# cloneofsimo/vqgan-training

Hardware: AMD Instinct MI355X
Metric: images/sec full train step (enc+dec+LPIPS+disc+bwd), 256x256 f=8 (higher is better)
Workload: dtype mixed like the reference: encoder+LPIPS+discriminator fp16 operands (TF32's 10-bit mantissa) / fp32 accumulate, decoder bf16

## Files before the change

### vqgan-training_amd/csrc/conv_wgrad.hip

```cpp
#include "vq_common.h"

struct WgradParams {
  VqConvDesc d;
  const void* x;
  const void* dy;
  float* part;
  float* bias_part;
  int dbg;
  int M, HoWo, RS;
  int n_ct, n_cit;
  int dsh, ush;
  int pix_per_split;
  int nsplit;
  int xcd_tiles;
  int wo_shift, ho_shift;
  int seg_shift;
  int x3;
};

#ifdef VQ_STAMPS_ON
__device__ long long g_vq_wstamps[64];
__device__ int g_vq_wstamp_n;
#define VQ_WSTAMP(id) do { if (blockIdx.x == 0 && threadIdx.x == 0) { const long long t_ = (long long)__builtin_readcyclecounter(); \
    const int k_ = g_vq_wstamp_n; if (k_ < 64) { g_vq_wstamps[k_] = ((long long)(id) << 56) | (t_ & 0x00ffffffffffffffll); g_vq_wstamp_n = k_ + 1; } } } while (0)
// ... 297 lines not shown
#pragma unroll
  for (int e = 0; e < 8; ++e) ones[e] = (short)One16<DT>::BITS;
#pragma unroll
  for (int e = 0; e < 16; ++e) bacc[e] = 0.f;

  const int gg = lane >> 4, tl = lane & 15;
  const int frow = 8 * (gg >> 1) + (tl >> 2);
  const int fcol = (gg & 1) * 16 + (tl & 3) * 4;
  auto frag_addr = [&](int chan0) -> int {
    const int c = chan0 + fcol;
    const int seg = (c * 2) >> 6, within = (c * 2) & 63;
    return frow * RB + ((seg ^ seg_key(frow)) << 6) + within;
  };
  auto frag_addr_x3 = [&](int chan0, int plane) -> int {
    const int c = chan0 + ((fcol >> 3) << 4) + (fcol & 7);
    const int seg = (c * 2) >> 6, within = ((c * 2) & 63) ^ ((seg & 1) << 4);
    return (frow * RB + ((seg ^ seg_key(frow)) << 6) + within) ^ (plane << 4);
  };
  int ya[FRC], xa[FRI];
#pragma unroll
  for (int a = 0; a < FRC; ++a) ya[a] = X3 ? frag_addr_x3(wco + (a >> 1) * 64, a & 1) : frag_addr(wco + a * 32);
#pragma unroll
  for (int b = 0; b < FRI; ++b) xa[b] = TILE * 2 + (X3 ? frag_addr_x3(wci + (b >> 1) * 64, b & 1) : frag_addr(wci + b * 32));
  constexpr int NRD = 2 * (FRC + FRI);
  static_assert(NRD <= 15, "lgkmcnt is a 4-bit counter");

  constexpr bool DB = BT < 256;
  auto run = [&](auto bias_tag) {
    constexpr bool BIAS = decltype(bias_tag)::value;
    s16x4 fy[DB ? 2 : 1][FRC][2], fx[DB ? 2 : 1][FRI][2];
    auto issue = [&](const char* base, auto kk_tag, int slot) {
      constexpr int KOFF = decltype(kk_tag)::value * 16 * RB;
#pragma unroll
      for (int a = 0; a < FRC; ++a) {
        fy[slot][a][0] = lds_read_tr16_b64_async<KOFF>(base + ya[a]);
        fy[slot][a][1] = lds_read_tr16_b64_async<KOFF + 4 * RB>(base + ya[a]);
      }
#pragma unroll
      for (int b = 0; b < FRI; ++b) {
        fx[slot][b][0] = lds_read_tr16_b64_async<KOFF>(base + xa[b]);
        fx[slot][b][1] = lds_read_tr16_b64_async<KOFF + 4 * RB>(base + xa[b]);
      }
    };
    auto mma = [&](int slot) {
#pragma unroll
      for (int a = 0; a < FRC; ++a)
#pragma unroll
        for (int h = 0; h < 2; ++h) vq_tie(fy[slot][a][h]);
#pragma unroll
      for (int b = 0; b < FRI; ++b)
#pragma unroll
        for (int h = 0; h < 2; ++h) vq_tie(fx[slot][b][h]);
      s16x8 af[FRC], bfr[FRI];
#pragma unroll
      for (int a = 0; a < FRC; ++a)
#pragma unroll
        for (int e = 0; e < 4; ++e) { af[a][e] = fy[slot][a][0][e]; af[a][4 + e] = fy[slot][a][1][e]; }
#pragma unroll
      for (int b = 0; b < FRI; ++b)
#pragma unroll
        for (int e = 0; e < 4; ++e) { bfr[b][e] = fx[slot][b][0][e]; bfr[b][4 + e] = fx[slot][b][1][e]; }
      if constexpr (X3) {
#pragma unroll
        for (int a = 0; a < AFR; ++a)
#pragma unroll
          for (int b = 0; b < BFR; ++b) {
            acc[a][b] = mfma16<DT>(af[2 * a], bfr[2 * b], acc[a][b]);
            acc[a][b] = mfma16<DT>(af[2 * a], bfr[2 * b + 1], acc[a][b]);
            acc[a][b] = mfma16<DT>(af[2 * a + 1], bfr[2 * b], acc[a][b]);
          }
        if constexpr (BIAS) {
          s16x8 selh = af[0], sell = af[1];
#pragma unroll
          for (int a = 1; a < AFR; ++a)
#pragma unroll
            for (int e = 0; e < 8; ++e) { selh[e] = (bias_frag == a) ? af[2 * a][e] : selh[e]; sell[e] = (bias_frag == a) ? af[2 * a + 1][e] : sell[e]; }
          bacc = mfma16<DT>(selh, ones, bacc);
          bacc = mfma16<DT>(sell, ones, bacc);
        }
      } else {
#pragma unroll
        for (int a = 0; a < FRC; ++a)
#pragma unroll
          for (int b = 0; b < FRI; ++b) acc[a][b] = mfma16<DT>(af[a], bfr[b], acc[a][b]);
        if constexpr (BIAS) {
          s16x8 sel = af[0];
#pragma unroll
          for (int a = 1; a < FRC; ++a)
#pragma unroll
            for (int e = 0; e < 8; ++e) sel[e] = (bias_frag == a) ? af[a][e] : sel[e];
          bacc = mfma16<DT>(sel, ones, bacc);
        }
      }
    };
    stage(0);
    wait_vmcnt<0>();
    raw_barrier();
    for (int c = 0; c < nchunks; ++c) {
      const char* base = (const char*)(lds + (c & 1) * 2 * TILE);
      issue(base, std::integral_constant<int, 0>{}, 0);
#ifdef VQ_ABLATION_KERNELS
      if (c + 1 < nchunks && !(p.dbg & 1)) stage((c + 1) & 1);
#else
      if (c + 1 < nchunks) stage((c + 1) & 1);
#endif
      if constexpr (DB) {
        issue(base, std::integral_constant<int, 1>{}, 1);
        wait_lgkmcnt<NRD>(); mma(0);
        issue(base, std::integral_constant<int, 2>{}, 0);
        wait_lgkmcnt<NRD>(); mma(1);
        issue(base, std::integral_constant<int, 3>{}, 1);
        wait_lgkmcnt<NRD>(); mma(0);
        wait_lgkmcnt<0>(); mma(1);
      } else {
        wait_lgkmcnt<0>(); mma(0);
        issue(base, std::integral_constant<int, 1>{}, 0);
        wait_lgkmcnt<0>(); mma(0);
        issue(base, std::integral_constant<int, 2>{}, 0);
        wait_lgkmcnt<0>(); mma(0);
        issue(base, std::integral_constant<int, 3>{}, 0);
        wait_lgkmcnt<0>(); mma(0);
      }
      wait_vmcnt<0>();
      raw_barrier();
    }
  };
  if (nchunks > 0) {
    if (do_bias) run(std::true_type{});
    else run(std::false_type{});
  }

  const int fr = lane & 31, fh = lane >> 5;
  const int CoutS = X3 ? p.d.Cout / 2 : p.d.Cout, CinS = X3 ? p.d.Cin / 2 : p.d.Cin;
  const int cob = X3 ? (co0 + wco) / 2 : co0 + wco, cib = X3 ? (ci0 + wci) / 2 : ci0 + wci;
  if (do_bias && (wave % NWI) == 0 && fr == 0) {
#pragma unroll
    for (int e = 0; e < 16; ++e)
      p.bias_part[(int64_t)split * CoutS + cob + bias_frag * 32 + (e & 3) + 8 * (e >> 2) + 4 * fh] = bacc[e];
  }
  float* out = p.part + ((int64_t)(split * p.RS + tap) * CoutS) * CinS;
#pragma unroll
  for (int a = 0; a < AFR; ++a)
#pragma unroll
    for (int b = 0; b < BFR; ++b) {
      const int ci = cib + b * 32 + fr;
#pragma unroll
      for (int e = 0; e < 16; ++e) {
        const int co = cob + a * 32 + (e & 3) + 8 * (e >> 2) + 4 * fh;
        wg_store(p, &out[(int64_t)co * CinS + ci], acc[a][b][e]);
      }
    }
}

template <int DT, int GEN, int NW, int SEG = 0, int STAG = 0, int X3 = 0>
__global__ __launch_bounds__(NW * 64, 2) void conv_wgrad3_kernel(const WgradParams p) {
  constexpr int BT = 128, BKP = 64, RB = BT * 2, XROWS = GEN ? 96 : 72;
  static_assert(GEN ? SEG == 0 : (SEG >= 4 && SEG <= 6), "SEG: compile-time segment shift of the power-of-two form");
  static_assert(!X3 || (NW == 4 && DT == VQ_F16), "the native three-product form: 2 x 2 waves over binary16 pieces");
  constexpr int TILE_Y = BKP * BT, TILE_X = XROWS * BT, STAGE = TILE_Y + TILE_X;
  constexpr int NWI = NW / 2, WTI = BT / NWI;
  constexpr int FRC = 2, FRI = WTI / 32;
  constexpr int AFR = X3 ? 1 : FRC, BFR = X3 ? 1 : FRI;
  constexpr int BXOR = X3 ? 4 : 6;
  static_assert(!X3 || FRI == 2, "native form: 64 virtual = 32 real channels per wave and side");
  constexpr int YP = (BKP / 4) / NW;
  constexpr int XPT = XROWS / 4, XP = (XPT + NW - 1) / NW;
  static_assert(NW == 4 || NW == 8, "2 x 2 or 2 x 4 waves");
  VQ_DYN_LDS(vq_bf16, lds);

  const int tid = threadIdx.x, lane = tid & 63, wave = tid >> 6;
  VQ_WSTAMP(20);
  const int wco = (wave / NWI) * 64, wci = (wave % NWI) * WTI;
  const int tiles = 3 * p.n_cit * p.n_ct;
  const int xcd = blockIdx.x & 7, jb = blockIdx.x >> 3;
  int split, t;
  if (p.xcd_tiles == 2) {
    const int per = (int)(gridDim.x >> 3), idx = xcd * per + jb;
    if (idx >= p.nsplit * tiles) return;
    split = idx / tiles;
    t = idx - split * tiles;
  } else if (p.xcd_tiles) {
    const int tpx = tiles >> 3;
    t = xcd * tpx + jb % tpx;
    split = jb / tpx;
  } else {
    split = (jb / tiles) * 8 + xcd;
    t = jb % tiles;
  }
  if (split >= p.nsplit) return;
  const int kr = t % 3; t /= 3;
  const int cit = t % p.n_cit; const int ct = t / p.n_cit;
  const int co0 = ct * BT, ci0 = cit * BT;
  const int pbeg = split * p.pix_per_split;
  int pend = pbeg + p.pix_per_split;
  if (pend > p.M) pend = p.M;
  const int nchunks = pbeg < pend ? (pend - pbeg + BKP - 1) / BKP : 0;

  const int W = p.d.Wo, H = p.d.Ho;
  const int wsh = p.wo_shift, hsh = p.ho_shift, wmask = W - 1, hmask = H - 1;
  constexpr bool pow2 = !GEN;
  const int segsh = GEN ? p.seg_shift : SEG;
  const int wseg = 1 << segsh, nslots = (BKP >> segsh) * (wseg + 2);
  const vq_bf16* zero = (const vq_bf16*)g_vq_wg_zero_page;
  const vq_bf16* dyb = (const vq_bf16*)p.dy;
  const vq_bf16* xb = (const vq_bf16*)p.x;

  const int lrow = lane >> 4, lp = lane & 15;
  auto lsl_of = [&](int row) -> int {
    const int seg = (lp >> 2) ^ (row & 3), gr = (lp & 3) ^ (X3 ? (seg & 1) : 0);
    return ((seg << 2) | gr) << 3;
  };
  const vq_bf16* pdy0 = dyb + (int64_t)(pbeg + wave * 4 + lrow) * p.d.Cout + co0 + lsl_of(lrow);
  const int dy_piece = 4 * NW * p.d.Cout;
  int xqj[GEN ? XP : 1];
  const int xlsl = lsl_of(lrow);
  if constexpr (GEN) {
#pragma unroll
    for (int i = 0; i < XP; ++i) {
      const int slot = (wave + NW * i) * 4 + lrow;
      const int q = slot / (wseg + 2);
      xqj[i] = slot < nslots ? ((q << 8) | (slot - q * (wseg + 2))) : -1;
    }
  }
  const int cin0 = ci0 + xlsl;
  int m0 = pbeg;
  auto stage = [&](int buf) {
    vq_bf16* ybase = lds + buf * STAGE;
    vq_bf16* xbase = ybase + TILE_Y;
#pragma unroll
    for (int i = 0; i < YP; ++i) glds16(pdy0 + i * dy_piece, ybase + (wave + NW * i) * 4 * BT);
    pdy0 += (int64_t)BKP * p.d.Cout;
#pragma unroll
    for (int i = 0; i < XP; ++i) {
      if (wave + NW * i < XPT) {
        int q, jj;
        bool have;
        if constexpr (GEN) { q = xqj[i] >> 8; jj = xqj[i] & 255; have = xqj[i] >= 0; }
        else {
          constexpr int WS2 = (1 << SEG) + 2;
          const int slot = (wave + NW * i) * 4 + lrow;
          q = slot / WS2; jj = slot - q * WS2; have = slot < (BKP >> SEG) * WS2;
        }
        const int ms = m0 + (q << segsh);
        int ox0, oy, n;
        if constexpr (pow2) { ox0 = ms & wmask; oy = (ms >> wsh) & hmask; n = ms >> (wsh + hsh); }
        else { n = ms / p.HoWo; const int rem = ms - n * p.HoWo; oy = rem / W; ox0 = rem - oy * W; }
        const int iy = oy + kr - 1, ix = ox0 - 1 + jj;
        const bool ok = have && (unsigned)iy < (unsigned)H && (unsigned)ix < (unsigned)W;
        const int off = ((n * p.d.H + (iy >> p.ush)) * p.d.W + (ix >> p.ush)) * p.d.Cin + cin0;
        const vq_bf16* src = ok ? xb + off : zero + xlsl;
        glds16((const void*)src, xbase + (wave + NW * i) * 4 * BT);
      }
    }
    m0 += BKP;
  };

  const int gg = lane >> 4, tl = lane & 15;
  const int frow = 8 * (gg >> 1) + (tl >> 2);
  const int fcol = (gg & 1) * 16 + (tl & 3) * 4;
  const int fcolv = X3 ? ((fcol >> 3) << 4) + (fcol & 7) : fcol;
  int ya[FRC];
#pragma unroll
  for (int a = 0; a < FRC; ++a) {
    const int c = wco + (X3 ? 0 : a * 32) + fcolv, seg = (c * 2) >> 6, within = ((c * 2) & 63) ^ (X3 ? ((seg & 1) << 4) : 0);
    ya[a] = (frow * RB + ((seg ^ (frow & 3)) << 6) + within) ^ (X3 ? (a << 4) : 0);
  }
  int xoff[GEN ? 4 : 1][GEN ? 3 : 1][GEN ? 2 : 1];
  int xsw[GEN ? 1 : 4];
  {
    const int c = wci + fcolv, seg = (c * 2) >> 6, within = ((c * 2) & 63) ^ (X3 ? ((seg & 1) << 4) : 0);
    if constexpr (GEN) {
#pragma unroll
      for (int kk = 0; kk < 4; ++kk)
#pragma unroll
        for (int ks = 0; ks < 3; ++ks)
#pragma unroll
          for (int h = 0; h < 2; ++h) {
            const int r = kk * 16 + frow + 4 * h;
            const int row = r + 2 * (r >> segsh) + ks;
            xoff[kk][ks][h] = TILE_Y * 2 + row * RB + ((seg ^ (row & 3)) << 6) + within;
          }
    } else {
#pragma unroll
      for (int j = 0; j < 4; ++j) xsw[j] = TILE_Y * 2 + frow * RB + ((seg ^ ((frow + j) & 3)) << 6) + within;
    }
  }

  f32x16 acc[3][AFR][BFR];
#pragma unroll
  for (int ks = 0; ks < 3; ++ks)
#pragma unroll
    for (int a = 0; a < AFR; ++a)
#pragma unroll
      for (int b = 0; b < BFR; ++b)
#pragma unroll
        for (int e = 0; e < 16; ++e) acc[ks][a][b][e] = 0.f;
  const bool do_bias = p.bias_part != nullptr && cit == 0 && kr < AFR;
  auto store_bias = [&](const f32x16& bacc) {
    const int fr_ = lane & 31, fh_ = lane >> 5;
    if ((wave % NWI) == 0 && fr_ == 0) {
      const int cob = X3 ? (co0 + wco) / 2 : co0 + wco + kr * 32, cstride = X3 ? p.d.Cout / 2 : p.d.Cout;
#pragma unroll
      for (int e = 0; e < 16; ++e)
        p.bias_part[(int64_t)split * cstride + cob + (e & 3) + 8 * (e >> 2) + 4 * fh_] = bacc[e];
    }
  };

  auto run = [&](auto bias_tag) {
    constexpr bool BIAS = decltype(bias_tag)::value;
    f32x16 bacc;
    s16x8 ones;
    if constexpr (BIAS) {
#pragma unroll
      for (int e = 0; e < 8; ++e) ones[e] = (short)One16<DT>::BITS;
#pragma unroll
      for (int e = 0; e < 16; ++e) bacc[e] = 0.f;
    }
    constexpr int NX = 2;
    s16x4 fy[2][FRC][2], fx[NX][FRI][2];
    auto issue_y = [&](const char* base, auto kk_tag) {
      constexpr int KK = decltype(kk_tag)::value, KOFF = KK * 16 * RB;
#pragma unroll
      for (int a = 0; a < FRC; ++a) {
        fy[KK & 1][a][0] = lds_read_tr16_b64_async<KOFF>(base + ya[a]);
        fy[KK & 1][a][1] = lds_read_tr16_b64_async<KOFF + 4 * RB>(base + ya[a]);
      }
    };
    auto issue_x = [&](const char* base, auto u_tag) {
      constexpr int U = decltype(u_tag)::value, KK = U / 3, KS = U % 3;
#pragma unroll
      for (int b = 0; b < FRI; ++b) {
        if constexpr (GEN) {
          fx[U % NX][b][0] = lds_read_tr16_b64_async<0>(base + (xoff[KK][KS][0] ^ (b << BXOR)));
          fx[U % NX][b][1] = lds_read_tr16_b64_async<0>(base + (xoff[KK][KS][1] ^ (b << BXOR)));
        } else {
          constexpr int UR = 16 * KK + 2 * (KK >> (SEG - 4)) + KS;
          fx[U % NX][b][0] = lds_read_tr16_b64_async<UR * RB>(base + (xsw[UR & 3] ^ (b << BXOR)));
          fx[U % NX][b][1] = lds_read_tr16_b64_async<(UR + 4) * RB>(base + (xsw[UR & 3] ^ (b << BXOR)));
        }
      }
    };
    auto step = [&](const char* base, auto u_tag) {
      constexpr int U = decltype(u_tag)::value, KK = U / 3, KS = U % 3;
      constexpr int NU = U + 1, NKK = NU / 3, NKS = NU % 3;
      if constexpr (NU < 12) {
        if constexpr (NKS == 0) issue_y(base, std::integral_constant<int, NKK>{});
        issue_x(base, std::integral_constant<int, NU>{});
        wait_lgkmcnt<(NKS == 0 ? 2 * FRC + 2 * FRI : 2 * FRI)>();
      } else {
        wait_lgkmcnt<0>();
      }
#pragma unroll
      for (int b = 0; b < FRI; ++b) vq_tie(fx[U % NX][b][0], fx[U % NX][b][1]);
      if constexpr (KS == 0) {
#pragma unroll
        for (int a = 0; a < FRC; ++a) vq_tie(fy[KK & 1][a][0], fy[KK & 1][a][1]);
      }
      s16x8 af[FRC], bfr[FRI];
#pragma unroll
      for (int a = 0; a < FRC; ++a)
#pragma unroll
        for (int e = 0; e < 4; ++e) { af[a][e] = fy[KK & 1][a][0][e]; af[a][4 + e] = fy[KK & 1][a][1][e]; }
#pragma unroll
      for (int b = 0; b < FRI; ++b)
#pragma unroll
        for (int e = 0; e < 4; ++e) { bfr[b][e] = fx[U % NX][b][0][e]; bfr[b][4 + e] = fx[U % NX][b][1][e]; }
      if constexpr (X3) {
        acc[KS][0][0] = mfma16<DT>(af[0], bfr[0], acc[KS][0][0]);
        acc[KS][0][0] = mfma16<DT>(af[0], bfr[1], acc[KS][0][0]);
        acc[KS][0][0] = mfma16<DT>(af[1], bfr[0], acc[KS][0][0]);
        if constexpr (BIAS && KS == 0) { bacc = mfma16<DT>(af[0], ones, bacc); bacc = mfma16<DT>(af[1], ones, bacc); }
      } else {
#pragma unroll
        for (int a = 0; a < FRC; ++a)
#pragma unroll
          for (int b = 0; b < FRI; ++b) acc[KS][a][b] = mfma16<DT>(af[a], bfr[b], acc[KS][a][b]);
        if constexpr (BIAS && KS == 0) bacc = mfma16<DT>(kr == 0 ? af[0] : af[1], ones, bacc);
      }
    };
    stage(0);
    wait_vmcnt<0>();
    raw_barrier();
    VQ_WSTAMP(21);
    for (int c = 0; c < nchunks; ++c) {
      const char* base = (const char*)(lds + (c & 1) * STAGE);
      issue_y(base, std::integral_constant<int, 0>{});
      issue_x(base, std::integral_constant<int, 0>{});
      const bool more = c + 1 < nchunks;
      const bool late = (STAG & 1) && wave >= NW / 2;
      if (more && !late) stage((c + 1) & 1);
      step(base, std::integral_constant<int, 0>{});  step(base, std::integral_constant<int, 1>{});
      step(base, std::integral_constant<int, 2>{});  step(base, std::integral_constant<int, 3>{});
      step(base, std::integral_constant<int, 4>{});  step(base, std::integral_constant<int, 5>{});
      if (more && late) stage((c + 1) & 1);
      step(base, std::integral_constant<int, 6>{});  step(base, std::integral_constant<int, 7>{});
      step(base, std::integral_constant<int, 8>{});  step(base, std::integral_constant<int, 9>{});
      step(base, std::integral_constant<int, 10>{}); step(base, std::integral_constant<int, 11>{});
      wait_vmcnt<0>();
      raw_barrier();
    }
    if constexpr (BIAS) store_bias(bacc);
  };
  if (nchunks > 0) {
    if (do_bias) run(std::true_type{});
    else run(std::false_type{});
  }
  VQ_WSTAMP(22);

  const int fr = lane & 31, fh = lane >> 5;
  const int CoutS = X3 ? p.d.Cout / 2 : p.d.Cout, CinS = X3 ? p.d.Cin / 2 : p.d.Cin;
  const int cob = X3 ? (co0 + wco) / 2 : co0 + wco, cib = X3 ? (ci0 + wci) / 2 : ci0 + wci;
#pragma unroll
  for (int ks = 0; ks < 3; ++ks) {
    float* out = p.part + ((int64_t)(split * p.RS + kr * 3 + ks) * CoutS) * CinS;
#pragma unroll
    for (int b = 0; b < BFR; ++b) {
      const int ci = cib + b * 32 + fr;
#pragma unroll
      for (int a = 0; a < AFR; ++a)
#pragma unroll
        for (int e = 0; e < 16; ++e) {
          const int co = cob + a * 32 + (e & 3) + 8 * (e >> 2) + 4 * fh;
          wg_store(p, &out[(int64_t)co * CinS + ci], acc[ks][a][b][e]);
        }
    }
  }
  VQ_WSTAMP(23);
}

__global__ void wgrad_reduce_kernel(const float* __restrict__ part, int nsplit, int RS, int Cout, int Cin,
                                    int Cout_w, int Cin_w, int accumulate, float* __restrict__ dw,
                                    const float* __restrict__ bias_part, float* __restrict__ dbias, int dw_blocks,
                                    float alpha, const float* __restrict__ alpha_dev) {
  if (alpha_dev) alpha *= *alpha_dev;
  if ((int)blockIdx.x >= dw_blocks) {
    const int c = ((int)blockIdx.x - dw_blocks) * blockDim.x + threadIdx.x;
    if (c < Cout_w) {
      float s = 0.f;
      for (int sp = 0; sp < nsplit; ++sp) s += bias_part[(int64_t)sp * Cout + c];
      s *= alpha;
      dbias[c] = accumulate ? dbias[c] + s : s;
    }
    return;
  }
  const int64_t per_tap = (int64_t)Cout_w * Cin_w, total = per_tap * RS;
  const int64_t plane = (int64_t)Cout * Cin;
  for (int64_t i = (int64_t)blockIdx.x * blockDim.x + threadIdx.x; i < total; i += (int64_t)dw_blocks * blockDim.x) {
    const int tap = (int)(i / per_tap);
    const int64_t j = i - (int64_t)tap * per_tap;
    const int co = (int)(j / Cin_w), ci = (int)(j - (int64_t)co * Cin_w);
    const float* src = part + (int64_t)tap * plane + (int64_t)co * Cin + ci;
    float s = 0.f;
    for (int sp = 0; sp < nsplit; ++sp) s += src[(int64_t)sp * RS * plane];
    s *= alpha;
    float* dst = dw + j * RS + tap;
    *dst = accumulate ? (*dst + s) : s;
  }
}

template <int LPI>
__global__ __launch_bounds__(256) void wgrad_reduce4_kernel(const float* __restrict__ part, int nsplit, int RS, int Cout, int Cin,
                                                            int Cout_w, int Cin_w, int accumulate, float* __restrict__ dw,
                                                            const float* __restrict__ bias_part, float* __restrict__ dbias,
                                                            int dw_blocks, float alpha, const float* __restrict__ alpha_dev) {
  if (alpha_dev) alpha *= *alpha_dev;
  if ((int)blockIdx.x >= dw_blocks) {
    const int c = ((int)blockIdx.x - dw_blocks) * blockDim.x + threadIdx.x;
    if (c < Cout_w) {
      float s = 0.f;
      for (int sp = 0; sp < nsplit; ++sp) s += bias_part[(int64_t)sp * Cout + c];
      s *= alpha;
      dbias[c] = accumulate ? dbias[c] + s : s;
    }
    return;
  }
  const int cq = Cin_w >> 2;
  const int64_t per_tap = (int64_t)Cout_w * cq, total = per_tap * RS;
  const int64_t plane = (int64_t)Cout * Cin, stride = (int64_t)RS * plane;
  const int sub = threadIdx.x % LPI;
  constexpr int IPB = 256 / LPI;
  const int64_t rounds = (total + (int64_t)dw_blocks * IPB - 1) / ((int64_t)dw_blocks * IPB);
  for (int64_t r = 0; r < rounds; ++r) {
    const int64_t i0 = (r * dw_blocks + blockIdx.x) * IPB + threadIdx.x / LPI;
    const bool live = i0 < total;
    const int64_t i = live ? i0 : total - 1;
    const int tap = (int)(i / per_tap);
    const int64_t j = i - (int64_t)tap * per_tap;
    const int co = (int)(j / cq), ci = (int)(j - (int64_t)co * cq) << 2;
    const float* src = part + (int64_t)tap * plane + (int64_t)co * Cin + ci;
    float4 s = make_float4(0.f, 0.f, 0.f, 0.f);
    int sp = sub;
    for (; sp + 7 * LPI < nsplit; sp += 8 * LPI) {
      float4 v[8];
#pragma unroll
      for (int u = 0; u < 8; ++u) v[u] = *(const float4*)(src + (int64_t)(sp + u * LPI) * stride);
#pragma unroll
      for (int u = 0; u < 8; ++u) { s.x += v[u].x; s.y += v[u].y; s.z += v[u].z; s.w += v[u].w; }
    }
    for (; sp < nsplit; sp += LPI) {
      const float4 v = *(const float4*)(src + (int64_t)sp * stride);
      s.x += v.x; s.y += v.y; s.z += v.z; s.w += v.w;
    }
#pragma unroll
    for (int m = 1; m < LPI; m <<= 1) {
      s.x += __shfl_xor(s.x, m); s.y += __shfl_xor(s.y, m); s.z += __shfl_xor(s.z, m); s.w += __shfl_xor(s.w, m);
    }
    if (live && sub == 0) {
      float* dst = dw + ((int64_t)co * Cin_w + ci) * RS + tap;
      const float rr[4] = {s.x * alpha, s.y * alpha, s.z * alpha, s.w * alpha};
#pragma unroll
      for (int k = 0; k < 4; ++k) dst[(int64_t)k * RS] = accumulate ? dst[(int64_t)k * RS] + rr[k] : rr[k];
    }
  }
}

__global__ __launch_bounds__(256) void wgrad_reduce9_kernel(const float* __restrict__ part, int nsplit, int Cout, int Cin, int Cout_w,
                                                            int Cin_w, int accumulate, float* __restrict__ dw,
                                                            const float* __restrict__ bias_part, float* __restrict__ dbias,
                                                            int dw_blocks, float alpha, const float* __restrict__ alpha_dev) {
  if (alpha_dev) alpha *= *alpha_dev;
  if ((int)blockIdx.x >= dw_blocks) {
    const int c = ((int)blockIdx.x - dw_blocks) * blockDim.x + threadIdx.x;
    if (c < Cout_w) {
      float s = 0.f;
      for (int sp = 0; sp < nsplit; ++sp) s += bias_part[(int64_t)sp * Cout + c];
      s *= alpha;
      dbias[c] = accumulate ? dbias[c] + s : s;
    }
    return;
  }
  const int cq = Cin_w >> 2;
  const int64_t total = (int64_t)Cout_w * cq;
  const int64_t plane = (int64_t)Cout * Cin, stride = 9 * plane;
  for (int64_t j = (int64_t)blockIdx.x * blockDim.x + threadIdx.x; j < total; j += (int64_t)dw_blocks * blockDim.x) {
    const int co = (int)(j / cq), ci = (int)(j - (int64_t)co * cq) << 2;
    const float* src = part + (int64_t)co * Cin + ci;
    float4 s[9];
#pragma unroll
    for (int t = 0; t < 9; ++t) s[t] = make_float4(0.f, 0.f, 0.f, 0.f);
    int sp = 0;
    for (; sp + 2 <= nsplit; sp += 2) {
      float4 v[2][9];
#pragma unroll
      for (int u = 0; u < 2; ++u)
#pragma unroll
        for (int t = 0; t < 9; ++t) v[u][t] = *(const float4*)(src + (int64_t)(sp + u) * stride + (int64_t)t * plane);
#pragma unroll
      for (int u = 0; u < 2; ++u)
#pragma unroll
        for (int t = 0; t < 9; ++t) { s[t].x += v[u][t].x; s[t].y += v[u][t].y; s[t].z += v[u][t].z; s[t].w += v[u][t].w; }
    }
    for (; sp < nsplit; ++sp) {
#pragma unroll
      for (int t = 0; t < 9; ++t) {
        const float4 v = *(const float4*)(src + (int64_t)sp * stride + (int64_t)t * plane);
        s[t].x += v.x; s[t].y += v.y; s[t].z += v.z; s[t].w += v.w;
      }
    }
    float r[36];
#pragma unroll
    for (int t = 0; t < 9; ++t) { r[t] = s[t].x * alpha; r[9 + t] = s[t].y * alpha; r[18 + t] = s[t].z * alpha; r[27 + t] = s[t].w * alpha; }
    float4* dst = (float4*)(dw + ((int64_t)co * Cin_w + ci) * 9);
#pragma unroll
    for (int q = 0; q < 9; ++q) {
      float4 o = make_float4(r[q * 4], r[q * 4 + 1], r[q * 4 + 2], r[q * 4 + 3]);
      if (accumulate) { const float4 old = dst[q]; o.x += old.x; o.y += old.y; o.z += old.z; o.w += old.w; }
      dst[q] = o;
    }
  }
}

template <int LPI>
__global__ __launch_bounds__(256) void wgrad_reduce_x2_kernel(const float* __restrict__ part, int nsplit, int RS, int CoutV, int CinV,
                                                              int Cout_w, int Cin_w, int accumulate, float* __restrict__ dw,
                                                              const float* __restrict__ bias_part, float* __restrict__ dbias,
                                                              int dw_blocks, float alpha, const float* __restrict__ alpha_dev) {
  if (alpha_dev) alpha *= *alpha_dev;
  if ((int)blockIdx.x >= dw_blocks) {
    const int c = ((int)blockIdx.x - dw_blocks) * blockDim.x + threadIdx.x;
    if (c < Cout_w) {
      const int vh = ((c >> 3) << 4) + (c & 7);
      float s = 0.f, t = 0.f;
      for (int sp = 0; sp < nsplit; ++sp) { s += bias_part[(int64_t)sp * CoutV + vh]; t += bias_part[(int64_t)sp * CoutV + vh + 8]; }
      s = (s + t) * alpha;
      dbias[c] = accumulate ? dbias[c] + s : s;
    }
    return;
  }
  const int cq = (Cin_w + 3) >> 2;
  const int64_t per_tap = (int64_t)Cout_w * cq, total = per_tap * RS;
  const int64_t plane = (int64_t)CoutV * CinV, stride = (int64_t)RS * plane;
  const int sub = threadIdx.x % LPI;
  constexpr int IPB = 256 / LPI;
  const int64_t rounds = (total + (int64_t)dw_blocks * IPB - 1) / ((int64_t)dw_blocks * IPB);
  for (int64_t r = 0; r < rounds; ++r) {
    const int64_t i0 = (r * dw_blocks + blockIdx.x) * IPB + threadIdx.x / LPI;
    const bool live = i0 < total;
    const int64_t i = live ? i0 : total - 1;
    const int tap = (int)(i / per_tap);
    const int64_t j = i - (int64_t)tap * per_tap;
    const int co = (int)(j / cq), ci = (int)(j - (int64_t)co * cq) << 2;
    const int vr = ((co >> 3) << 4) + (co & 7), vc = ((ci >> 3) << 4) + (ci & 7);
    const float* src = part + (int64_t)tap * plane + (int64_t)vr * CinV + vc;
    const int64_t lo_row = (int64_t)8 * CinV;
    float4 big = make_float4(0.f, 0.f, 0.f, 0.f), small = make_float4(0.f, 0.f, 0.f, 0.f);
    for (int sp = sub; sp < nsplit; sp += LPI) {
      const float* q = src + (int64_t)sp * stride;
      const float4 hh = *(const float4*)q, hl = *(const float4*)(q + 8), lh = *(const float4*)(q + lo_row), ll = *(const float4*)(q + lo_row + 8);
      big.x += hh.x; big.y += hh.y; big.z += hh.z; big.w += hh.w;
      small.x += (hl.x + lh.x) + ll.x; small.y += (hl.y + lh.y) + ll.y; small.z += (hl.z + lh.z) + ll.z; small.w += (hl.w + lh.w) + ll.w;
    }
#pragma unroll
    for (int m = 1; m < LPI; m <<= 1) {
      big.x += __shfl_xor(big.x, m); big.y += __shfl_xor(big.y, m); big.z += __shfl_xor(big.z, m); big.w += __shfl_xor(big.w, m);
      small.x += __shfl_xor(small.x, m); small.y += __shfl_xor(small.y, m); small.z += __shfl_xor(small.z, m); small.w += __shfl_xor(small.w, m);
    }
    if (live && sub == 0) {
      float* dst = dw + ((int64_t)co * Cin_w + ci) * RS + tap;
      const float rr[4] = {(big.x + small.x) * alpha, (big.y + small.y) * alpha, (big.z + small.z) * alpha, (big.w + small.w) * alpha};
#pragma unroll
      for (int k = 0; k < 4; ++k)
        if (ci + k < Cin_w) dst[(int64_t)k * RS] = accumulate ? dst[(int64_t)k * RS] + rr[k] : rr[k];
    }
  }
}
static inline VqConvDesc wg_x2_virtual(const VqConvDesc* d) {
  VqConvDesc v = *d;
  if (v.dtype == VQ_F16X2) { v.dtype = VQ_F16; v.Cin *= 2; v.Cout *= 2; v.Cin_w = v.Cin; v.Cout_w = v.Cout; }
  return v;
}

static int ilog2_exact_w(int v) {
  int s = 0;
  while ((1 << s) < v) ++s;
  return ((1 << s) == v) ? s : -1;
}

static bool wgrad_glds_eligible(const VqConvDesc* d) {
  return (d->dtype == VQ_BF16 || d->dtype == VQ_F16) && d->split == 1 && ilog2_exact_w(d->Wo) >= 0 && ilog2_exact_w(d->Ho) >= 0 &&
         ((int64_t)d->N * d->Ho * d->Wo) % 64 == 0 && d->Cout % 64 == 0 && d->Cin % 64 == 0;
}

static inline int wg_hint_tile(const VqConvDesc* d) { return d->kernel_hint & (64 | 128 | 256); }
static inline bool wg_hint_no3(const VqConvDesc* d) { return (d->kernel_hint & 4) != 0; }
static inline bool wg_hint_slow_reduce(const VqConvDesc* d) { return (d->kernel_hint & 1) != 0; }
static inline bool wg_hint_unstaggered(const VqConvDesc* d) { return (d->kernel_hint & 16) != 0; }
static inline int wg_hint_split(const VqConvDesc* d) { return (d->kernel_hint >> 16) & 0xffff; }
static inline bool wg_hint_x2_virtual(const VqConvDesc* d) { return (d->kernel_hint & 8) != 0; }
static bool wg_hint_supported(const VqConvDesc* d) { return (d->kernel_hint & 0xffff & ~(1 | 4 | 8 | 16 | 64 | 128 | 256)) == 0; }

static bool wgrad3_eligible(const VqConvDesc* d) {
  return (d->dtype == VQ_BF16 || d->dtype == VQ_F16) && d->split == 1 && ((int64_t)d->N * d->Ho * d->Wo) % 64 == 0 && !wg_hint_no3(d) && !wg_hint_tile(d) &&
         d->R == 3 && d->S == 3 && d->stride == 1 && d->dil_in == 1 && (d->up == 1 || d->up == 2) && d->pad_t == 1 &&
         d->pad_l == 1 && d->Ho == d->H * d->up && d->Wo == d->W * d->up && d->Wo % 4 == 0 && d->Cout % 128 == 0 &&
         d->Cin % 128 == 0;
}

static int wgrad_cus() {
#ifdef VQ_ABLATION_KERNELS
  static const int v = [] { const char* e = getenv("VQ_WGRAD_CUS"); const int x = e ? atoi(e) : 0; return (x >= 8 && x <= 256) ? x / 8 * 8 : 256; }();
  return v;
#else
  return 256;
#endif
}
static void wgrad_plan(const VqConvDesc* d, int& BT, int& n_ct, int& n_cit, int& nsplit, int& pix_per_split, int* xcd_tiles = nullptr,
                       bool x3 = false) {
  if (xcd_tiles) *xcd_tiles = 0;
  BT = (d->Cout >= 128 && d->Cin >= 128) ? 128 : 64;
  if (wgrad_glds_eligible(d)) {
    if (d->Cout % 256 == 0 && d->Cin % 256 == 0 &&
        (int64_t)d->N * d->Ho * d->Wo >= (d->R * d->S >= 16 ? 16384 : 131072)) BT = 256;
    else if (d->Cout % 128 == 0 && d->Cin % 128 == 0) BT = 128;
    else BT = 64;
    if (wg_hint_tile(d) && d->Cout % wg_hint_tile(d) == 0 && d->Cin % wg_hint_tile(d) == 0) BT = wg_hint_tile(d);
  }
  const bool three = wgrad3_eligible(d);
  if (three) BT = 128;
  n_ct = (int)vq_ceil_div(d->Cout, BT);
  n_cit = (int)vq_ceil_div(d->Cin, BT);
  const int64_t M = (int64_t)d->N * d->Ho * d->Wo;
  const int tiles = n_ct * n_cit * (three ? 3 : d->R * d->S);
  const bool one_per_cu = (BT == 256 || three) && !x3;
  const int cus = wgrad_cus();
  int64_t want = vq_ceil_div((one_per_cu ? 2 : 3) * cus, tiles);
  int64_t max_split = vq_ceil_div(M, 512);
  if (want > max_split) want = max_split;
  if (want < 1) want = 1;
  if (want > 256) want = 256;
  if ((wgrad_glds_eligible(d) || three) && max_split >= 8) want = vq_ceil_div(want, 8) * 8;
  if ((wgrad_glds_eligible(d) || three) && max_split >= 8) {
    const int slots = cus * (one_per_cu ? 1 : (BT == 128 ? 2 : 4));
    const double t_kernel = 2.0 * (double)M * d->Cout * d->Cin * d->R * d->S / 7.0e14;
    const double t_split = 2.0 * d->R * d->S * d->Cout * d->Cin * 4.0 / 4.0e12 * (x3 ? 0.25 : 1.0);
    double best = 1e30;
    for (int64_t ns = 8; ns <= max_split && ns <= 256; ns += 8) {
      const int64_t blocks = ns * tiles, rounds = vq_ceil_div(blocks, slots);
      const double cost = t_kernel * (double)(rounds * slots) / (double)blocks + t_split * (double)ns;
      if (cost < best) { best = cost; want = ns; }
    }
    if (xcd_tiles) {
      const int mode = (three && tiles % 8 == 0) ? 1 : 2;
      if (mode == 2 || tiles % 8 == 0) {
        for (int64_t ns = 1; ns <= max_split && ns <= 256; ++ns) {
          const int64_t blocks = ns * tiles, rounds = vq_ceil_div(blocks, slots);
          const double cost = t_kernel * (double)(rounds * slots) / (double)blocks + t_split * (double)ns;
          if (cost < best * 0.97) { best = cost; want = ns; *xcd_tiles = mode; }
        }
      }
    }
  }
  if (xcd_tiles && *xcd_tiles == 0 && (three || wgrad_glds_eligible(d)) && want % 8 != 0) *xcd_tiles = 2;
  if (wg_hint_split(d) > 0) {
    want = wg_hint_split(d) < max_split ? wg_hint_split(d) : max_split;
    if (xcd_tiles) *xcd_tiles = ((three || wgrad_glds_eligible(d)) && want % 8 != 0) ? ((three && tiles % 8 == 0) ? 1 : 2) : 0;
  }
  int64_t pps = vq_ceil_div(vq_ceil_div(M, want), 64) * 64;
  nsplit = (int)vq_ceil_div(M, pps);
  pix_per_split = (int)pps;
}

static size_t wgrad_part_bytes(const VqConvDesc* d, int nsplit) {
  return (size_t)nsplit * d->R * d->S * d->Cout * d->Cin * sizeof(float);
}
static size_t wgrad_bias_bytes(const VqConvDesc* d, int nsplit) {
  return ((size_t)nsplit * d->Cout * sizeof(float) + 255) / 256 * 256;
}
static bool wg_x3(const VqConvDesc* d0, const VqConvDesc* dvirt) {
  return d0->dtype == VQ_F16X2 && !wg_hint_x2_virtual(d0) && wgrad3_eligible(dvirt);
}
static bool wg_x3_glds(const VqConvDesc* d0, const VqConvDesc* dvirt, int BT) {
  return d0->dtype == VQ_F16X2 && !wg_hint_x2_virtual(d0) && !wgrad3_eligible(dvirt) && wgrad_glds_eligible(dvirt) && BT >= 128;
}

template <int DT, int BT, int NW, int X3 = 0>
static int launch_wgrad_glds(const WgradParams& p, dim3 grid, hipStream_t s) {
  constexpr size_t LDS_BYTES = (size_t)2 * 2 * 64 * BT * sizeof(vq_bf16);
  VQ_RESERVE_LDS((conv_wgrad_glds_kernel<DT, BT, NW, X3>), LDS_BYTES, "vq_conv2d_wgrad");
  hipLaunchKernelGGL((conv_wgrad_glds_kernel<DT, BT, NW, X3>), grid, dim3(NW * 64), LDS_BYTES, s, p);
  return VQ_OK;
}

template <int DT, int GEN, int NW, int SEG, int STAG, int X3 = 0>
static int launch_wgrad3_form(const WgradParams& p, dim3 grid, hipStream_t s) {
  constexpr size_t LDS_BYTES = (size_t)2 * (64 + (GEN ? 96 : 72)) * 128 * sizeof(vq_bf16);
  static_assert(LDS_BYTES <= 160 * 1024, "LDS capacity");
  VQ_RESERVE_LDS((conv_wgrad3_kernel<DT, GEN, NW, SEG, STAG, X3>), LDS_BYTES, "vq_conv2d_wgrad");
  hipLaunchKernelGGL((conv_wgrad3_kernel<DT, GEN, NW, SEG, STAG, X3>), grid, dim3(NW * 64), LDS_BYTES, s, p);
  return VQ_OK;
}
template <int DT, int GEN, int NW, int STAG, int X3 = 0>
static int launch_wgrad3_nw(const WgradParams& p, dim3 grid, hipStream_t s) {
  if constexpr (GEN) return launch_wgrad3_form<DT, 1, NW, 0, STAG, X3>(p, grid, s);
  else {
    if (p.seg_shift == 4) return launch_wgrad3_form<DT, 0, NW, 4, STAG, X3>(p, grid, s);
    if (p.seg_shift == 5) return launch_wgrad3_form<DT, 0, NW, 5, STAG, X3>(p, grid, s);
    return launch_wgrad3_form<DT, 0, NW, 6, STAG, X3>(p, grid, s);
  }
}
template <int DT, int GEN>
static int launch_wgrad3(const WgradParams& p, dim3 grid, hipStream_t s) {
  if ((int64_t)p.d.N * p.d.H * p.d.W * p.d.Cin >= ((int64_t)1 << 31)) { vq_set_error("vq_conv2d_wgrad(three-tap): input of 2^31 elements or more"); return VQ_ERR_UNSUPPORTED; }
  if constexpr (DT == VQ_F16) {
    if (p.x3) return launch_wgrad3_nw<DT, GEN, 4, 1, 1>(p, grid, s);
  }
  if (!wg_hint_unstaggered(&p.d)) return launch_wgrad3_nw<DT, GEN, 8, 1>(p, grid, s);
  return launch_wgrad3_nw<DT, GEN, 8, 0>(p, grid, s);
}

extern "C" size_t vq_conv2d_wgrad_workspace(const VqConvDesc* d0) {
  if (!d0) return 0;
  if (vq_wgrad_c8_x2_eligible(d0))
    return (vq_wgrad_c8_x2_workspace(d0) + 255) / 256 * 256 + vq_colsum_workspace((int64_t)d0->N * d0->Ho * d0->Wo, d0->Cout);
  const VqConvDesc dvirt = wg_x2_virtual(d0);
  const VqConvDesc* d = &dvirt;
  int BT, n_ct, n_cit, nsplit, pps;
  int xt;
  bool x3 = wg_x3(d0, d);
  wgrad_plan(d, BT, n_ct, n_cit, nsplit, pps, &xt, x3);
  x3 = x3 || wg_x3_glds(d0, d, BT);
  size_t main_bytes = x3 ? wgrad_part_bytes(d0, nsplit) + wgrad_bias_bytes(d0, nsplit)
                         : wgrad_part_bytes(d, nsplit) + wgrad_bias_bytes(d, nsplit);
  if (vq_wgrad_c8_eligible(d)) main_bytes = (vq_wgrad_c8_workspace(d) + 255) / 256 * 256;
  return main_bytes + vq_colsum_workspace((int64_t)d->N * d->Ho * d->Wo, d->Cout);
}

extern "C" int vq_conv2d_wgrad(const VqConvDesc* d0, const void* x, const void* dy, float* dw, float* dbias, int accumulate,
                               void* workspace, size_t ws_bytes, void* stream) {
  VQ_REQUIRE(d0 && x && dy && dw, VQ_ERR_INVALID, "vq_conv2d_wgrad: null pointer");
  const bool x2 = d0->dtype == VQ_F16X2;
  VQ_REQUIRE(!x2 || d0->split == 1, VQ_ERR_UNSUPPORTED, "vq_conv2d_wgrad: VQ_F16X2 storage takes split = 1");
  const VqConvDesc dvirt = wg_x2_virtual(d0);
  const VqConvDesc* d = &dvirt;
  VQ_REQUIRE(d->Cin % 8 == 0 && d->Cout % 8 == 0, VQ_ERR_INVALID, "vq_conv2d_wgrad: channels must be multiples of 8");
  const int dsh = ilog2_exact_w(d->dil_in), ush = ilog2_exact_w(d->up);
  VQ_REQUIRE(dsh >= 0 && ush >= 0 && ush <= 1, VQ_ERR_UNSUPPORTED, "vq_conv2d_wgrad: bad dil_in/up");
  VQ_REQUIRE(d->subpix == 0, VQ_ERR_UNSUPPORTED, "vq_conv2d_wgrad: sub-pixel descriptors are forward-only");
  VQ_REQUIRE(wg_hint_supported(d), VQ_ERR_UNSUPPORTED, "vq_conv2d_wgrad: unknown kernel_hint bits (%d)", d->kernel_hint);
  VQ_REQUIRE((int64_t)d->N * d->Ho * d->Wo < (1ll << 31) - 4096, VQ_ERR_UNSUPPORTED, "vq_conv2d_wgrad: pixel count exceeds int32");
  const size_t need = vq_conv2d_wgrad_workspace(d0);
  VQ_REQUIRE(workspace && ws_bytes >= need, VQ_ERR_WORKSPACE, "vq_conv2d_wgrad: workspace too small (%zu < %zu)", ws_bytes, need);
  const float alpha = d->alpha == 0.f ? 1.f : d->alpha;
  if (vq_wgrad_c8_x2_eligible(d0)) {
    int bias_done = 0;
    int rc = vq_launch_wgrad_c8_x2(d0, x, dy, dw, dbias, &bias_done, accumulate, alpha, workspace, (hipStream_t)stream);
    if (rc) return rc;
    if (dbias && !bias_done) {
      const int64_t pixels = (int64_t)d0->N * d0->Ho * d0->Wo;
      void* cws = (char*)workspace + (vq_wgrad_c8_x2_workspace(d0) + 255) / 256 * 256;
      return vq_colsum(dy, pixels, d0->Cout, d0->dtype, dbias, d0->Cout_w, accumulate, alpha, nullptr, cws,
                       vq_colsum_workspace(pixels, d0->Cout), stream);
    }
    return VQ_OK;
  }
  if (vq_wgrad_c8_eligible(d)) {
    VQ_REQUIRE(d->alpha_dev == nullptr, VQ_ERR_UNSUPPORTED, "vq_conv2d_wgrad: the 8-channel kernels take a host alpha only");
    int bias_done = 0;
    int rc = vq_launch_wgrad_c8(d, x, dy, dw, dbias, &bias_done, accumulate, alpha, workspace, (hipStream_t)stream);
    if (rc) return rc;
    if (dbias && !bias_done) {
      const int64_t pixels = (int64_t)d->N * d->Ho * d->Wo;
      void* cws = (char*)workspace + (vq_wgrad_c8_workspace(d) + 255) / 256 * 256;
      return vq_colsum(dy, pixels, d->Cout, d->dtype, dbias, d->Cout_w, accumulate, alpha, nullptr, cws,
                       vq_colsum_workspace(pixels, d->Cout), stream);
    }
    return VQ_OK;
  }
  WgradParams p;
  p.d = *d; p.x = x; p.dy = dy; p.part = (float*)workspace;
  p.M = d->N * d->Ho * d->Wo; p.HoWo = d->Ho * d->Wo; p.RS = d->R * d->S;
  p.dsh = dsh; p.ush = ush;
  int BT, nsplit;
  bool x3 = wg_x3(d0, d);
  wgrad_plan(d, BT, p.n_ct, p.n_cit, nsplit, p.pix_per_split, &p.xcd_tiles, x3);
  x3 = x3 || wg_x3_glds(d0, d, BT);
  p.x3 = x3 ? 1 : 0;
  hipStream_t s = (hipStream_t)stream;
  dim3 grid(p.n_ct * p.n_cit * p.RS, nsplit);
  p.wo_shift = ilog2_exact_w(d->Wo); p.ho_shift = ilog2_exact_w(d->Ho);
  const bool glds_ok = wgrad_glds_eligible(d) || wgrad3_eligible(d);
  p.seg_shift = 0;
  while (p.seg_shift < 6 && d->Wo % (2 << p.seg_shift) == 0) ++p.seg_shift;
  const VqConvDesc* ds = x3 ? d0 : d;
  float* bias_part = (float*)((char*)workspace + wgrad_part_bytes(ds, nsplit));
  void* colsum_ws = (char*)bias_part + wgrad_bias_bytes(ds, nsplit);
  p.bias_part = (glds_ok && dbias && (wgrad3_eligible(d) || p.RS * p.n_cit >= BT / 64)) ? bias_part : nullptr;
#define VQ_WG(DTv, SPv, BTv, NB) \
  hipLaunchKernelGGL((conv_wgrad_kernel<DTv, SPv, BTv, 32, NB>), grid, dim3(256), 0, s, p)
  p.nsplit = nsplit;
#ifdef VQ_ABLATION_KERNELS
  p.dbg = wg_hint_slow_reduce(d) ? 1 : 0;
#else
  p.dbg = 0;
#endif
  if (glds_ok) {
    int rc = VQ_OK;
    const bool three = wgrad3_eligible(d);
    const dim3 grid1(p.xcd_tiles == 2 ? 8u * (unsigned)vq_ceil_div((int64_t)nsplit * (p.n_ct * p.n_cit * (three ? 3 : p.RS)), 8)
                     : p.xcd_tiles ? (unsigned)nsplit * (unsigned)(p.n_ct * p.n_cit * 3)
                                 : 8u * (unsigned)vq_ceil_div(nsplit, 8) * (unsigned)(p.n_ct * p.n_cit * (three ? 3 : p.RS)));
    const bool pow2 = p.wo_shift >= 0 && p.ho_shift >= 0 && d->Wo >= 16;
    if (d->dtype == VQ_F16) {
      if (three) rc = pow2 ? launch_wgrad3<VQ_F16, 0>(p, grid1, s) : launch_wgrad3<VQ_F16, 1>(p, grid1, s);
      else if (BT == 256) rc = p.x3 ? launch_wgrad_glds<VQ_F16, 256, 8, 1>(p, grid1, s) : launch_wgrad_glds<VQ_F16, 256, 8>(p, grid1, s);
      else if (BT == 128) rc = p.x3 ? launch_wgrad_glds<VQ_F16, 128, 4, 1>(p, grid1, s) : launch_wgrad_glds<VQ_F16, 128, 4>(p, grid1, s);
      else rc = launch_wgrad_glds<VQ_F16, 64, 4>(p, grid1, s);
    } else {
      if (three) rc = pow2 ? launch_wgrad3<VQ_BF16, 0>(p, grid1, s) : launch_wgrad3<VQ_BF16, 1>(p, grid1, s);
      else if (BT == 256) rc = launch_wgrad_glds<VQ_BF16, 256, 8>(p, grid1, s);
      else if (BT == 128) rc = launch_wgrad_glds<VQ_BF16, 128, 4>(p, grid1, s);
      else rc = launch_wgrad_glds<VQ_BF16, 64, 4>(p, grid1, s);
    }
    if (rc) return rc;
  } else if (d->dtype == VQ_BF16 && d->split == 1) {
    if (BT == 128) VQ_WG(VQ_BF16, 1, 128, 2); else VQ_WG(VQ_BF16, 1, 64, 2);
  } else if (d->dtype == VQ_F16 && d->split == 1) {
    if (BT == 128) VQ_WG(VQ_F16, 1, 128, 2); else VQ_WG(VQ_F16, 1, 64, 2);
  } else if (d->dtype == VQ_F32 && d->split == 1) {
    if (BT == 128) VQ_WG(VQ_F32, 1, 128, 2); else VQ_WG(VQ_F32, 1, 64, 2);
  } else if (d->dtype == VQ_F32 && d->split == 3) {
    if (BT == 128) VQ_WG(VQ_F32, 3, 128, 1); else VQ_WG(VQ_F32, 3, 64, 1);
  } else if (d->dtype == VQ_F32 && d->split == 6) {
    if (BT == 128) VQ_WG(VQ_F32, 6, 128, 1); else VQ_WG(VQ_F32, 6, 64, 1);
  } else {
    vq_set_error("vq_conv2d_wgrad: unsupported dtype/split combination (%d/%d)", d->dtype, d->split);
    return VQ_ERR_UNSUPPORTED;
  }
#undef VQ_WG
  VQ_CHECK_LAUNCH("vq_conv2d_wgrad");
  d = ds;
  const int64_t total = (int64_t)d->Cout_w * d->Cin_w * p.RS;
  int blocks = (int)vq_ceil_div(total, 256);
  if (blocks > 4096) blocks = 4096;
  const int bias_blocks = (dbias && p.bias_part) ? (d->Cout_w + 255) / 256 : 0;
  if (x2 && !x3) {
    const int64_t items = (int64_t)d0->Cout_w * ((d0->Cin_w + 3) / 4) * p.RS;
    int lpi = 1;
    while (lpi < 8 && items * lpi < 131072 && lpi * 2 <= nsplit) lpi *= 2;
    blocks = (int)vq_ceil_div(items * lpi, 256);
    if (blocks > 4096) blocks = 4096;
    const int bb = (dbias && p.bias_part) ? (d0->Cout_w + 255) / 256 : 0;
#define VQ_RX(L) hipLaunchKernelGGL(wgrad_reduce_x2_kernel<L>, dim3(blocks + bb), dim3(256), 0, s, (const float*)workspace, nsplit, p.RS, \
                       d->Cout, d->Cin, d0->Cout_w, d0->Cin_w, accumulate, dw, (const float*)bias_part, dbias, blocks, alpha, d->alpha_dev)
    if (lpi == 8) VQ_RX(8); else if (lpi == 4) VQ_RX(4); else if (lpi == 2) VQ_RX(2); else VQ_RX(1);
#undef VQ_RX
  } else
  if (p.RS == 9 && d->Cin % 4 == 0 && d->Cin_w % 4 == 0 && (int64_t)d->Cout_w * d->Cin_w >= 512 * 512 && !wg_hint_slow_reduce(d) &&
      ((uintptr_t)dw & 15) == 0) {
    blocks = (int)vq_ceil_div((int64_t)d->Cout_w * (d->Cin_w / 4), 256);
    hipLaunchKernelGGL(wgrad_reduce9_kernel, dim3(blocks + bias_blocks), dim3(256), 0, s, (const float*)workspace, nsplit, d->Cout,
                       d->Cin, d->Cout_w, d->Cin_w, accumulate, dw, (const float*)bias_part, dbias, blocks, alpha, d->alpha_dev);
  } else if (d->Cin % 4 == 0 && d->Cin_w % 4 == 0 && !wg_hint_slow_reduce(d)) {
    const int64_t items = total / 4;
    int lpi = 1;
    while (lpi < 8 && items * lpi < 131072 && lpi * 2 <= nsplit) lpi *= 2;
    blocks = (int)vq_ceil_div(items * lpi, 256);
    if (blocks > 4096) blocks = 4096;
#define VQ_R4(L) hipLaunchKernelGGL(wgrad_reduce4_kernel<L>, dim3(blocks + bias_blocks), dim3(256), 0, s, (const float*)workspace, nsplit, p.RS, \
                       d->Cout, d->Cin, d->Cout_w, d->Cin_w, accumulate, dw, (const float*)bias_part, dbias, blocks, alpha, d->alpha_dev)
    if (lpi == 8) VQ_R4(8); else if (lpi == 4) VQ_R4(4); else if (lpi == 2) VQ_R4(2); else VQ_R4(1);
// ... 17 lines not shown
```

Before: 278.7.

## Add producer-wave specialization with triple-buffered LDS to three-tap wgrad kernel

Adds a warp-specialized form of the three-tap weight-gradient kernel in which four extra producer waves issue all global-to-LDS staging while the eight MFMA waves only compute. The LDS ring grows to three stages so producers can run up to two chunks ahead, waiting on vmcnt only for the older stage. This is now the default for non-GEN bf16/fp16 paths unless a hint disables it, replacing the staggered form. It targets load latency stalls in the compute waves, but it adds waves per block, raises LDS use to three stages, which may cut occupancy, and relies on barrier pairing between producers and consumers.

New measurement: 273.9. 1.7% lower.

```diff
diff --git a/vqgan-training_amd/csrc/conv_wgrad.hip b/vqgan-training_amd/csrc/conv_wgrad.hip
--- a/vqgan-training_amd/csrc/conv_wgrad.hip
+++ b/vqgan-training_amd/csrc/conv_wgrad.hip
@@ -473,8 +473,8 @@
     }
 }
 
-template <int DT, int GEN, int NW, int SEG = 0, int STAG = 0, int X3 = 0>
-__global__ __launch_bounds__(NW * 64, 2) void conv_wgrad3_kernel(const WgradParams p) {
+template <int DT, int GEN, int NW, int SEG = 0, int STAG = 0, int X3 = 0, int NP = 0, int NB = 2>
+__global__ __launch_bounds__((NW + NP) * 64, 2) void conv_wgrad3_kernel(const WgradParams p) {
   constexpr int BT = 128, BKP = 64, RB = BT * 2, XROWS = GEN ? 96 : 72;
   static_assert(GEN ? SEG == 0 : (SEG >= 4 && SEG <= 6), "SEG: compile-time segment shift of the power-of-two form");
   static_assert(!X3 || (NW == 4 && DT == VQ_F16), "the native three-product form: 2 x 2 waves over binary16 pieces");
@@ -484,12 +484,17 @@
   constexpr int AFR = X3 ? 1 : FRC, BFR = X3 ? 1 : FRI;
   constexpr int BXOR = X3 ? 4 : 6;
   static_assert(!X3 || FRI == 2, "native form: 64 virtual = 32 real channels per wave and side");
-  constexpr int YP = (BKP / 4) / NW;
-  constexpr int XPT = XROWS / 4, XP = (XPT + NW - 1) / NW;
   static_assert(NW == 4 || NW == 8, "2 x 2 or 2 x 4 waves");
+  static_assert(NP == 0 ? NB == 2 : (NW == 8 && !STAG && !X3 && (NP == 2 || NP == 4) && (NB == 2 || NB == 3)), "producer form: 8 MFMA waves + NP staging waves");
+  constexpr int SW = NP ? NP : NW;
+  constexpr int YP = (BKP / 4) / SW;
+  constexpr int XPT = XROWS / 4, XP = (XPT + SW - 1) / SW;
+  constexpr int PMIN = YP + XPT / SW;
   VQ_DYN_LDS(vq_bf16, lds);
 
   const int tid = threadIdx.x, lane = tid & 63, wave = tid >> 6;
+  const bool producer = NP && __builtin_amdgcn_readfirstlane(wave) >= NW;
+  const int sw = NP ? wave - NW : wave;
   VQ_WSTAMP(20);
   const int wco = (wave / NWI) * 64, wci = (wave % NWI) * WTI;
   const int tiles = 3 * p.n_cit * p.n_ct;
@@ -531,14 +536,14 @@
     const int seg = (lp >> 2) ^ (row & 3), gr = (lp & 3) ^ (X3 ? (seg & 1) : 0);
     return ((seg << 2) | gr) << 3;
   };
-  const vq_bf16* pdy0 = dyb + (int64_t)(pbeg + wave * 4 + lrow) * p.d.Cout + co0 + lsl_of(lrow);
-  const int dy_piece = 4 * NW * p.d.Cout;
+  const vq_bf16* pdy0 = dyb + (int64_t)(pbeg + sw * 4 + lrow) * p.d.Cout + co0 + lsl_of(lrow);
+  const int dy_piece = 4 * SW * p.d.Cout;
   int xqj[GEN ? XP : 1];
   const int xlsl = lsl_of(lrow);
   if constexpr (GEN) {
 #pragma unroll
     for (int i = 0; i < XP; ++i) {
-      const int slot = (wave + NW * i) * 4 + lrow;
+      const int slot = (sw + SW * i) * 4 + lrow;
       const int q = slot / (wseg + 2);
       xqj[i] = slot < nslots ? ((q << 8) | (slot - q * (wseg + 2))) : -1;
     }
@@ -549,17 +554,17 @@
     vq_bf16* ybase = lds + buf * STAGE;
     vq_bf16* xbase = ybase + TILE_Y;
 #pragma unroll
-    for (int i = 0; i < YP; ++i) glds16(pdy0 + i * dy_piece, ybase + (wave + NW * i) * 4 * BT);
+    for (int i = 0; i < YP; ++i) glds16(pdy0 + i * dy_piece, ybase + (sw + SW * i) * 4 * BT);
     pdy0 += (int64_t)BKP * p.d.Cout;
 #pragma unroll
     for (int i = 0; i < XP; ++i) {
-      if (wave + NW * i < XPT) {
+      if (sw + SW * i < XPT) {
         int q, jj;
         bool have;
         if constexpr (GEN) { q = xqj[i] >> 8; jj = xqj[i] & 255; have = xqj[i] >= 0; }
         else {
           constexpr int WS2 = (1 << SEG) + 2;
-          const int slot = (wave + NW * i) * 4 + lrow;
+          const int slot = (sw + SW * i) * 4 + lrow;
           q = slot / WS2; jj = slot - q * WS2; have = slot < (BKP >> SEG) * WS2;
         }
         const int ms = m0 + (q << segsh);
@@ -570,7 +575,7 @@
         const bool ok = have && (unsigned)iy < (unsigned)H && (unsigned)ix < (unsigned)W;
         const int off = ((n * p.d.H + (iy >> p.ush)) * p.d.W + (ix >> p.ush)) * p.d.Cin + cin0;
         const vq_bf16* src = ok ? xb + off : zero + xlsl;
-        glds16((const void*)src, xbase + (wave + NW * i) * 4 * BT);
+        glds16((const void*)src, xbase + (sw + SW * i) * 4 * BT);
       }
     }
     m0 += BKP;
@@ -699,15 +704,19 @@
         if constexpr (BIAS && KS == 0) bacc = mfma16<DT>(kr == 0 ? af[0] : af[1], ones, bacc);
       }
     };
-    stage(0);
-    wait_vmcnt<0>();
+    if constexpr (NP == 0) {
+      stage(0);
+      wait_vmcnt<0>();
+    }
     raw_barrier();
     VQ_WSTAMP(21);
+    int buf = 0;
     for (int c = 0; c < nchunks; ++c) {
-      const char* base = (const char*)(lds + (c & 1) * STAGE);
+      const char* base = (const char*)(lds + buf * STAGE);
+      buf = buf + 1 == NB ? 0 : buf + 1;
       issue_y(base, std::integral_constant<int, 0>{});
       issue_x(base, std::integral_constant<int, 0>{});
-      const bool more = c + 1 < nchunks;
+      const bool more = NP == 0 && c + 1 < nchunks;
       const bool late = (STAG & 1) && wave >= NW / 2;
       if (more && !late) stage((c + 1) & 1);
       step(base, std::integral_constant<int, 0>{});  step(base, std::integral_constant<int, 1>{});
@@ -717,16 +726,35 @@
       step(base, std::integral_constant<int, 6>{});  step(base, std::integral_constant<int, 7>{});
       step(base, std::integral_constant<int, 8>{});  step(base, std::integral_constant<int, 9>{});
       step(base, std::integral_constant<int, 10>{}); step(base, std::integral_constant<int, 11>{});
-      wait_vmcnt<0>();
+      if constexpr (NP == 0) wait_vmcnt<0>();
       raw_barrier();
     }
     if constexpr (BIAS) store_bias(bacc);
   };
+  auto produce = [&]() {
+    stage(0);
+    if (NB == 3 && nchunks > 1) { stage(1); wait_vmcnt<PMIN>(); }
+    else wait_vmcnt<0>();
+    raw_barrier();
+    int buf = NB - 1;
+    for (int c = 0; c < nchunks; ++c) {
+      if (c + NB - 1 < nchunks) {
+        stage(buf);
+        buf = buf + 1 == NB ? 0 : buf + 1;
+        if constexpr (NB == 3) wait_vmcnt<PMIN>(); else wait_vmcnt<0>();
+      } else {
+        wait_vmcnt<0>();
+      }
+      raw_barrier();
+    }
+  };
   if (nchunks > 0) {
-    if (do_bias) run(std::true_type{});
+    if (producer) produce();
+    else if (do_bias) run(std::true_type{});
     else run(std::false_type{});
   }
   VQ_WSTAMP(22);
+  if (producer) return;
 
   const int fr = lane & 31, fh = lane >> 5;
   const int CoutS = X3 ? p.d.Cout / 2 : p.d.Cout, CinS = X3 ? p.d.Cin / 2 : p.d.Cin;
@@ -968,7 +996,8 @@
 static inline bool wg_hint_unstaggered(const VqConvDesc* d) { return (d->kernel_hint & 16) != 0; }
 static inline int wg_hint_split(const VqConvDesc* d) { return (d->kernel_hint >> 16) & 0xffff; }
 static inline bool wg_hint_x2_virtual(const VqConvDesc* d) { return (d->kernel_hint & 8) != 0; }
-static bool wg_hint_supported(const VqConvDesc* d) { return (d->kernel_hint & 0xffff & ~(1 | 4 | 8 | 16 | 64 | 128 | 256)) == 0; }
+static inline bool wg_hint_no_producers(const VqConvDesc* d) { return (d->kernel_hint & 32) != 0; }
+static bool wg_hint_supported(const VqConvDesc* d) { return (d->kernel_hint & 0xffff & ~(1 | 4 | 8 | 16 | 32 | 64 | 128 | 256)) == 0; }
 
 static bool wgrad3_eligible(const VqConvDesc* d) {
   return (d->dtype == VQ_BF16 || d->dtype == VQ_F16) && d->split == 1 && ((int64_t)d->N * d->Ho * d->Wo) % 64 == 0 && !wg_hint_no3(d) && !wg_hint_tile(d) &&
@@ -1062,21 +1091,21 @@
   return VQ_OK;
 }
 
-template <int DT, int GEN, int NW, int SEG, int STAG, int X3 = 0>
+template <int DT, int GEN, int NW, int SEG, int STAG, int X3 = 0, int NP = 0, int NB = 2>
 static int launch_wgrad3_form(const WgradParams& p, dim3 grid, hipStream_t s) {
-  constexpr size_t LDS_BYTES = (size_t)2 * (64 + (GEN ? 96 : 72)) * 128 * sizeof(vq_bf16);
+  constexpr size_t LDS_BYTES = (size_t)NB * (64 + (GEN ? 96 : 72)) * 128 * sizeof(vq_bf16);
   static_assert(LDS_BYTES <= 160 * 1024, "LDS capacity");
-  VQ_RESERVE_LDS((conv_wgrad3_kernel<DT, GEN, NW, SEG, STAG, X3>), LDS_BYTES, "vq_conv2d_wgrad");
-  hipLaunchKernelGGL((conv_wgrad3_kernel<DT, GEN, NW, SEG, STAG, X3>), grid, dim3(NW * 64), LDS_BYTES, s, p);
+  VQ_RESERVE_LDS((conv_wgrad3_kernel<DT, GEN, NW, SEG, STAG, X3, NP, NB>), LDS_BYTES, "vq_conv2d_wgrad");
+  hipLaunchKernelGGL((conv_wgrad3_kernel<DT, GEN, NW, SEG, STAG, X3, NP, NB>), grid, dim3((NW + NP) * 64), LDS_BYTES, s, p);
   return VQ_OK;
 }
-template <int DT, int GEN, int NW, int STAG, int X3 = 0>
+template <int DT, int GEN, int NW, int STAG, int X3 = 0, int NP = 0, int NB = 2>
 static int launch_wgrad3_nw(const WgradParams& p, dim3 grid, hipStream_t s) {
-  if constexpr (GEN) return launch_wgrad3_form<DT, 1, NW, 0, STAG, X3>(p, grid, s);
+  if constexpr (GEN) return launch_wgrad3_form<DT, 1, NW, 0, STAG, X3, NP, NB>(p, grid, s);
   else {
-    if (p.seg_shift == 4) return launch_wgrad3_form<DT, 0, NW, 4, STAG, X3>(p, grid, s);
-    if (p.seg_shift == 5) return launch_wgrad3_form<DT, 0, NW, 5, STAG, X3>(p, grid, s);
-    return launch_wgrad3_form<DT, 0, NW, 6, STAG, X3>(p, grid, s);
+    if (p.seg_shift == 4) return launch_wgrad3_form<DT, 0, NW, 4, STAG, X3, NP, NB>(p, grid, s);
+    if (p.seg_shift == 5) return launch_wgrad3_form<DT, 0, NW, 5, STAG, X3, NP, NB>(p, grid, s);
+    return launch_wgrad3_form<DT, 0, NW, 6, STAG, X3, NP, NB>(p, grid, s);
   }
 }
 template <int DT, int GEN>
@@ -1085,8 +1114,9 @@
   if constexpr (DT == VQ_F16) {
     if (p.x3) return launch_wgrad3_nw<DT, GEN, 4, 1, 1>(p, grid, s);
   }
-  if (!wg_hint_unstaggered(&p.d)) return launch_wgrad3_nw<DT, GEN, 8, 1>(p, grid, s);
-  return launch_wgrad3_nw<DT, GEN, 8, 0>(p, grid, s);
+  if (wg_hint_unstaggered(&p.d)) return launch_wgrad3_nw<DT, GEN, 8, 0>(p, grid, s);
+  if (GEN || wg_hint_no_producers(&p.d)) return launch_wgrad3_nw<DT, GEN, 8, 1>(p, grid, s);
+  return launch_wgrad3_nw<DT, 0, 8, 0, 0, 4, 3>(p, grid, s);
 }
 
 extern "C" size_t vq_conv2d_wgrad_workspace(const VqConvDesc* d0) {
```
